# GiboDidact/Computational_ray_tracer

Hardware: AMD Instinct MI355X
Metric: Msamples/s (whole node) at 1920x1080; achieved HBM GB/s vs roofline (higher is better)
Workload: dtype f32; 1 GPU; BASELINE configs[1]: Cornell box 1920x1080 @ 256 spp (16x16 stratified jittered), diffuse + NEE, max depth 5, 1 quad light, 36 triangles; spp_total=256, max_depth=5, parallelism=pixel-tile shards x1 (32x32 tiles) + RCCL film reduce

## Files before the change

### computational_ray_tracer_amd/csrc/rt_host.cpp

```cpp
#include <algorithm>
#include <cstddef>
#include <cstdlib>
#include <cmath>
#include <cstdio>
#include <cstring>
#include <initializer_list>
#include <limits>
#include <queue>
#include <string>
#include <thread>
#include <utility>
#include <vector>

#include "../../include/rtmi355x.h"
#include "../data/spectra_data.h"
#include "../data/sensor_data.h"
#include "rt_devbuf.h"
#include "rt_guard.h"
#include "rt_internal.h"
#include "rt_texture.h"

using namespace rtmi;

namespace {
// ... 431 lines not shown
    hipStream_t stream = nullptr;
    hipEvent_t film_done = nullptr;
};

struct Knobs {
    bool stage_events = true;
    int lanes = kDefaultLanes;
    int shadow_queue = 0;
    int shadow_dfs = 1;
    int sort_rays = 1;
    float bvh_node_cost = 2.5f;
    int bvh_max_leaf = kBvhMaxLeaf;
    float bvh_any_cost = 2.f;
    int bvh_any_leaf = 4;
    int force_amb = -1;
    int coop = 1;
    int mat_bins = 1;
    int emit_filter = 1;
    int debug_path = 0;
    int sort_dir_bits = 3, sort_org_bits = 3;
    int sort_org_major = -1;
    int sort_nee = 1, sort_nee_bits = 8;
    int hit_compact = 1;
    size_t batch_samples = 0;
    int denoise_lds = 1;
};

static Knobs read_knobs() {
    Knobs k;
    if (std::getenv("RTMI_NO_STAGE_EVENTS")) k.stage_events = false;
    if (const char* e = std::getenv("RTMI_LANES")) k.lanes = std::max(1, std::min(kLanes, std::atoi(e)));
    if (const char* e = std::getenv("RTMI_SHADOW_QUEUE")) k.shadow_queue = std::atoi(e);
    if (const char* e = std::getenv("RTMI_SHADOW_DFS")) k.shadow_dfs = std::atoi(e);
    if (const char* e = std::getenv("RTMI_SORT")) k.sort_rays = std::atoi(e);
    if (const char* e = std::getenv("RTMI_BVH_CI")) k.bvh_node_cost = (float)std::atof(e);
    if (const char* e = std::getenv("RTMI_BVH_LEAF")) k.bvh_max_leaf = std::max(1, std::min(15, std::atoi(e)));
    if (const char* e = std::getenv("RTMI_BVH_ANY")) {
        float ac;
        int al;
        if (std::sscanf(e, "%f/%d", &ac, &al) == 2) {
            k.bvh_any_cost = ac;
            k.bvh_any_leaf = std::max(1, std::min(15, al));
        }
    }
    if (const char* e = std::getenv("RTMI_FORCE_AMB")) k.force_amb = std::max(-1, std::min(30, std::atoi(e)));
    if (const char* e = std::getenv("RTMI_COOP")) k.coop = std::atoi(e) != 0;
    if (const char* e = std::getenv("RTMI_MAT_BINS")) k.mat_bins = std::atoi(e);
    if (const char* e = std::getenv("RTMI_EMIT_FILTER")) k.emit_filter = std::atoi(e);
    if (const char* e = std::getenv("RTMI_DEBUG_PATH_KERNELS")) k.debug_path = std::atoi(e) != 0;
    if (const char* e = std::getenv("RTMI_SORT_BITS")) {
        int db = 3, ob = 4, om = -1;
        const int got = std::sscanf(e, "%d/%d/%d", &db, &ob, &om);
        if (got >= 2 && db >= 0 && db <= 9 && ob >= 0 && ob <= 9 && 3 + 2 * db + 3 * ob <= 32) {
            k.sort_dir_bits = db;
            k.sort_org_bits = ob;
            if (got == 3) k.sort_org_major = om < 0 ? -1 : (om ? 1 : 0);
        }
    }
    if (const char* e = std::getenv("RTMI_SORT_NEE")) std::sscanf(e, "%d/%d", &k.sort_nee, &k.sort_nee_bits);
    k.sort_nee_bits = std::max(1, std::min(9, k.sort_nee_bits));
    if (const char* e = std::getenv("RTMI_HIT_COMPACT")) k.hit_compact = std::atoi(e) != 0;
    if (const char* e = std::getenv("RTMI_BATCH_SAMPLES")) k.batch_samples = (size_t)std::max(0L, std::atol(e));
    if (const char* e = std::getenv("RTMI_DENOISE_LDS")) k.denoise_lds = std::atoi(e) != 0;
    return k;
}

struct rt_ctx {
    float4 sort_lo{}, sort_scale{};
    int device = 0;
    int octree_build = RT_OCTREE_BUILD_DEVICE;
    hipStream_t stream = nullptr;
    std::string err;
    bool have_scene = false, have_cam = false, have_smp = false, have_film = false, have_integ = false;
    rt_camera_desc cam{};
    rt_sampler_desc smp{};
    rt_film_desc film{};
    rt_integrator_desc integ{};
    int n_tris = 0;
    std::vector<float> h_bounds;
    std::vector<int32_t> h_child, h_leaf_first, h_leaf_count, h_refs;
    rt_octree_info info{};
    bool cull = false;
    bool scene_full = false;
    DevScene dsc{};
// ... 152 lines not shown
    HIPCHK(c, b.shLA.reserve(n)); HIPCHK(c, b.shLB.reserve(n));
    return RT_OK;
}

int ensure_sort_workspace(rt_ctx* c, Batch& b, size_t n) {
    HIPCHK(c, b.sRay.reserve(2 * n)); HIPCHK(c, b.sS.reserve(n));
    HIPCHK(c, b.sVals.reserve(n)); HIPCHK(c, b.sValsAlt.reserve(n));
    HIPCHK(c, b.sKeys.reserve(n)); HIPCHK(c, b.sKeysAlt.reserve(n)); HIPCHK(c, b.sQKey.reserve(n));
    HIPCHK(c, b.sTemp.reserve(sort_temp_bytes()));
    return RT_OK;
}

int ensure_ring(rt_ctx* c, Work& w) {
    if (c->dsc.qcap != 0) return RT_OK;
    HIPCHK(c, w.ring.reserve((size_t)c->dsc.ring_threads * (size_t)(c->dsc.ring_mask + 1)));
    return RT_OK;
}
DevScene lane_scene(const rt_ctx* c, const Work& w) {
    DevScene d = c->dsc;
    d.ring = w.ring.get();
    return d;
}

int ensure_workspace(rt_ctx* c, Work& w, size_t n, bool path) {
    int rc;
    HIPCHK(c, w.qcount.reserve(2 * kQRegion));
    if (&w != &c->ws[0] && !w.stream) HIPCHK(c, hipStreamCreateWithFlags(&w.stream, hipStreamNonBlocking));
    if (!w.film_done) HIPCHK(c, hipEventCreateWithFlags(&w.film_done, hipEventDisableTiming));
    if ((rc = ensure_ring(c, w))) return rc;
    Batch& b = w.b;
    const bool hit_d = path && c->knobs.hit_compact && c->dsc.qcap == 1 && !c->dsc.full;
    if (b.capacity(path) >= n) {
        if (hit_d) HIPCHK(c, b.hitD.reserve(n));
        return RT_OK;
    }
    b = Batch{};
    size_t nq = path ? 2 * n : n;
    HIPCHK(c, b.ray.reserve(2 * nq));
    HIPCHK(c, b.pdfA.reserve(n)); HIPCHK(c, b.pdfB.reserve(n));
    HIPCHK(c, b.hitB.reserve(n)); HIPCHK(c, b.hitPrim.reserve(n));
    if (path) {
        HIPCHK(c, b.rec.reserve((size_t)kRecF4 * n));
        if (hit_d) HIPCHK(c, b.hitD.reserve(n));
    } else {
        HIPCHK(c, b.lamA.reserve(n)); HIPCHK(c, b.lamB.reserve(n));
    }
    return RT_OK;
}

static int dim_get2d(const DevSampler& S, int dim) {
    if (S.kind == 1) return dim + 2;
    if (S.kind == 2) return (dim + 1 >= kSobolDims ? 2 : dim) + 2;
    return dim;
}
static int dim_after_camera(const DevSampler& S, const DevCamera& cam) {
    int dim = S.kind == 2 ? 2 : 0;
// ... 359 lines not shown
            int nIdx = std::min(B, ie - b0);
            int nS = nIdx * n_work;
            SampleIds ids = sample_ids(work, n_work, b0);
            RefIO r = ref_io(c, w.b, nS, nsh);
            hipEvent_t e0 = ev_start(c, st);
            HIPCHK(c, launch_generate(st, c->grid, nS, ids, cam, smp, fd, r.go));
            ev_mark(c, st, ST_GEN, e0);
            e0 = ev_start(c, st);
            HIPCHK(c, launch_trace_closest(st, 0, c->dsc.qcap, lane_scene(c, w), r.tio, d_ctr));
            ev_mark(c, st, ST_TRACE, e0);
            r.sio.work_pixels = work; r.sio.n_pixels = n_work; r.sio.n_index = nIdx;
            r.sio.film = film;
            r.sio.mom = pass.mom;
            e0 = ev_start(c, st);
            HIPCHK(c, launch_ref_shade_film(st, 0, c->dsc, d_spec, fd, r.sio, d_ctr));
            ev_mark(c, st, ST_FILM, e0);
        }
        return RT_OK;
    }

    const int nbatch = (ie - ib + B - 1) / B;
    const int lanes = std::max(1, std::min(std::min(kn.lanes, kLanes), nbatch));
    const bool sort_rays = c->dsc.qcap != 1 && kn.sort_rays;
    for (int l = 0; l < lanes; ++l) {
        if ((rc = ensure_workspace(c, c->ws[l], ncap, true))) return rc;
        if (sort_rays && (rc = ensure_sort_workspace(c, c->ws[l].b, ncap))) return rc;
        if (c->dsc.qcap != 1) HIPCHK(c, c->ws[l].tfb.reserve(ncap));
    }
    const bool dyn = c->dsc.qcap != 1;
    const int lean = c->dsc.full ? 2 : 1;
    const bool shq = c->dsc.qcap != 1 && !c->dsc.full;
    if (shq)
        for (int l = 0; l < lanes; ++l)
            if ((rc = ensure_shadow_workspace(c, c->ws[l].b, ncap))) return rc;
    const bool nee = c->dsc.full && c->dsc.n_lights > 0;
    if (nee)
        for (int l = 0; l < lanes; ++l)
            if ((rc = ensure_nee_workspace(c, c->ws[l].b, nmax * (size_t)nee_stride(c->dsc.n_lights), ncap))) return rc;
    const bool bins = nee && c->dsc.qcap != 1 && kn.mat_bins;
    const int grid = c->grid;
    auto lstream = [&](int l) { return l == 0 ? st : c->ws[l].stream; };
    if (lanes > 1) {
        HIPCHK(c, hipEventRecord(c->ws[0].film_done, st));
        for (int l = 1; l < lanes; ++l) HIPCHK(c, hipStreamWaitEvent(c->ws[l].stream, c->ws[0].film_done, 0));
    }
    const size_t qs = ncap;
    const bool records = c->dsc.qcap != 1;
    const size_t rec_fs = records ? 1 : nmax;
// ... 31 lines not shown
                int nxt = cur[l] ^ 1;
                const float4* cO = b.rayO() + 2 * (size_t)cur[l] * qs;
                const float4* cD = cO + 1;
                int* qc_cur = w.qcount.get() + kQRegion * cur[l];
                int* qc_nxt = w.qcount.get() + kQRegion * nxt;
                const bool efilter = kn.emit_filter && c->dsc.full && depth == c->integ.max_depth && depth > 0 &&
                                     c->dsc.n_emit_tris >= 0;
                if (efilter) HIPCHK(c, hipMemsetAsync(qc_nxt, 0, kQRegion * sizeof(int), s));
                hipEvent_t e0;
                QueueView qv = depth == 0 ? QueueView{nullptr, Sq[l], nSq[l], nsh}
                                          : QueueView{qc_cur + kQLen, Sq[l], 0, nsh};
                const DevScene dsl = lane_scene(c, w);
                if (efilter) {
                    const EmitIO eio{qv, cO, b.rayO() + 2 * (size_t)nxt * qs, qc_nxt + kQLen};
                    e0 = ev_start(c, s);
                    HIPCHK(c, launch_emitter_filter(s, grid, dsl, eio));
                    ev_mark(c, s, ST_FILTER, e0);
                    cO = eio.nO;
                    cD = cO + 1;
                    qv = QueueView{qc_nxt + kQLen, Sq[l], 0, nsh};
                }
                TraceIO tio{cO, cD, qv, 0, b.hitB.get(), b.hitPrim.get(), dyn ? qc_cur + kQTraceTicket : nullptr, 1};
                if (depth > 0 && !efilter) tio.zero = qc_nxt;
                const bool hitc = kn.hit_compact && c->dsc.qcap == 1 && !c->dsc.full && depth > 0;
                if (hitc) {
                    tio.hq_d = b.hitD.get();
                    tio.hq_len = qc_cur + kQShadowLen;
                }
                if (c->dsc.qcap != 1) {
                    tio.fb_pos = w.tfb.get();
                    tio.fb_len = qc_cur + kQTraceFallback;
                }
                const NeeSlots ns = nee ? b.nee : NeeSlots{};
                BinIO bio{qv, b.hitPrim.get(), {}, qc_cur + kQBinLen};
                for (int cl = 0; cl < kMatClasses; ++cl) bio.idx[cl] = ns.bin[cl];
                if (depth == 0) { bio.rayO = cO; bio.rec = rv; }
                if (sort_rays && depth > 0 && !efilter) {
                    SortRaysIO so{b.sQKey.get(), b.sS.get(), b.sKeys.get(), b.sKeysAlt.get(), b.sVals.get(),
                                  b.sValsAlt.get(), b.sTemp.get(), kn.sort_dir_bits, kn.sort_org_bits, qc_cur + kQLen,
                                  Sq[l]};
                    e0 = ev_start(c, s);
                    HIPCHK(c, launch_sort_rays(s, so));
                    ev_mark(c, s, ST_SORT, e0);
                    tio.perm = b.sS.get();
                    tio.so = b.sRay.get();
                    cO = tio.so; cD = cO + 1;
                }
                e0 = ev_start(c, s);
                HIPCHK(c, launch_trace_closest(s, grid, c->dsc.qcap, dsl, tio, d_ctr));
// ... 34 lines not shown
                    sqio.defer = kn.shadow_queue ? 0 : 1;
                }
                NeeIO nio{};
                const bool sort_nee = nee && sort_rays && kn.sort_nee;
                if (nee)
                    nio = NeeIO{b.neeRec.get(), ns.queue, qc_cur + kQShadowLen, qc_cur + kQShadowTicket, ns.fallback,
                                qc_cur + kQNeeFallback, sort_nee ? ns.key : nullptr, c->sort_lo, c->sort_scale,
                                kn.sort_nee_bits};
                if (c->tx.live) nio.tex = c->tx.dev.get();
                nio.ml = c->ml.any ? 1 : 0;
                e0 = ev_start(c, s);
                if (bins) {
                    HIPCHK(c, launch_bin_materials(s, grid, dsl, bio));
                    for (int cl = 0; cl < kMatClasses; ++cl) {
                        PathIO bp = pio;
                        bp.q = QueueView{qc_cur + kQBinLen + cl * kShards * kQStride, Sq[l], 0, nsh};
                        bp.ticket = qc_cur + kQBinTicket + cl * kShards * kQStride;
                        bp.bin_idx = bio.idx[cl];
                        HIPCHK(c, launch_path_shade(s, grid, c->dsc.qcap, dsl, d_spec, smp, fd, ids, bp, d_ctr,
                                                    sqio, nio, 1 + cl));
                    }
                } else {
                    HIPCHK(c, launch_path_shade(s, grid, c->dsc.qcap, dsl, d_spec, smp, fd, ids, pio, d_ctr, sqio,
                                                nio));
                }
                ev_mark(c, s, ST_SHADE, e0);
                if (sort_nee) {
                    SortNeeIO so{ns.queue, qc_cur + kQShadowLen, Sq[l], ns.key, b.sKeys.get(), b.sKeysAlt.get(),
                                 b.sVals.get(), b.sValsAlt.get(), b.sTemp.get(), kn.sort_nee_bits};
                    e0 = ev_start(c, s);
                    HIPCHK(c, launch_sort_nee(s, so));
                    ev_mark(c, s, ST_SORT, e0);
                }
                if (nee) {
                    e0 = ev_start(c, s);
                    HIPCHK(c, launch_path_nee(s, grid, c->dsc.qcap, dsl, d_spec, pio, nio, d_ctr));
                    if (c->dsc.qcap != 1 && !c->dsc.coop_ok)
                        HIPCHK(c, launch_path_nee_fallback(s, grid, c->dsc.qcap, dsl, d_spec, pio, nio, d_ctr));
                    ev_mark(c, s, ST_SHADOW, e0);
                }
                if (shq && !(sqio.defer && c->dsc.coop_ok)) {
                    e0 = ev_start(c, s);
                    HIPCHK(c, launch_path_shadow(s, grid, c->dsc.qcap, kn.shadow_dfs != 0, dsl, pio, sqio, d_ctr));
                    ev_mark(c, s, ST_SHADOW, e0);
                }
                cur[l] = nxt;
            }
// ... 2539 lines not shown
```

### computational_ray_tracer_amd/csrc/rt_internal.h

```cpp
#pragma once
#include <hip/hip_runtime.h>
#include <stdint.h>

#include <vector>

namespace rtmi {

static const int kSpecN = 471;
static const int kF1Max = 128;

struct DevSpectra {
    float X[kSpecN], Y[kSpecN], Z[kSpecN], D65[kSpecN];
    float f1_lambda[kF1Max], f1_value[kF1Max];
    int f1_n;
    float bk7_lambda[kF1Max], bk7_value[kF1Max];
    int bk7_n;
    float SR[kSpecN], SG[kSpecN], SB[kSpecN];
    float4 SPK[kSpecN];
};

struct DevCamera {
    float r2c[16], c2w[16];
    float lens_radius, focal_distance;
    int type;
// ... 192 lines not shown

static const int kShards = 8;
static const int kQStride = 64;
enum { kQLen = 0, kQTraceTicket = 1 * kShards * kQStride, kQShadeTicket = 2 * kShards * kQStride,
       kQShadowLen = 3 * kShards * kQStride, kQShadowTicket = 4 * kShards * kQStride,
       kQNeeFallback = 5 * kShards * kQStride,
       kQBinLen = 6 * kShards * kQStride, kQBinTicket = 8 * kShards * kQStride,
       kQTraceFallback = 10 * kShards * kQStride,
       kQRegion = 11 * kShards * kQStride };
static const int kMatClasses = 2;
inline __host__ __device__ int shard_stride(int n, int ns) {
    int s = (n + ns - 1) / ns;
    return (s + 63) & ~63;
}
struct QueueView {
    const int* len;
    int S;
    int n;
    int ns;
};
static const int kBlockThreads = 256;
static const int kClusterTris = 2;

struct TraceIO {
    const float4* rayO; const float4* rayD;
    QueueView q;
    int set;
    float4* hitB;
    int* hitPrim;
    int* ticket = nullptr;
    int rsh = 0;
    const int* perm = nullptr;
    float4* so = nullptr;
    int* fb_pos = nullptr;
    int* fb_len = nullptr;
    int* zero = nullptr;
    float4* hq_d = nullptr;
    int* hq_len = nullptr;
};

struct BinIO {
    QueueView q;
    const int* hitPrim;
    int* idx[kMatClasses];
    int* len;
    const float4* rayO = nullptr;
    RecView rec{};
};
hipError_t launch_bin_materials(hipStream_t st, int grid, const DevScene& sc, const BinIO& io);

struct EmitIO {
    QueueView q;
    const float4* rayO;
    float4* nO;
// ... 116 lines not shown
size_t sort_temp_bytes();
hipError_t launch_sort_rays(hipStream_t st, const SortRaysIO& io);
struct SortNeeIO {
    int* slot; int* len; int S;
    const unsigned* key;
    unsigned* keys; unsigned* keys_alt; int* vals; int* vals_alt;
    void* temp;
    int org_bits;
};
hipError_t launch_sort_nee(hipStream_t st, const SortNeeIO& io);
hipError_t launch_oct_classify(hipStream_t st, int nnodes, const float* cbox, const int* seg, const int* ent,
                               const float* tri9, unsigned char* mask, int* stats);
hipError_t launch_oct_scatter(hipStream_t st, int njobs, int nchild, const int* job, const int* ent,
                              const unsigned char* mask, int* ent_next, int* s0);
hipError_t launch_ref_shade_film(hipStream_t st, int grid, const DevScene& sc, const DevSpectra* sp, const DevFilm& film,
                                 const ShadeRefIO& io, unsigned long long* ctr);
hipError_t launch_records(hipStream_t st, const DevScene& sc, const DevSpectra* sp, const DevFilm& film,
                          const ShadeRefIO& sio, const RecordIO& io);
hipError_t launch_path_shadow(hipStream_t st, int grid, int qcap, bool dfs, const DevScene& sc, const PathIO& io,
                              const ShadowQueueIO& shq, unsigned long long* ctr);
hipError_t launch_path_shade(hipStream_t st, int grid, int qcap, const DevScene& sc, const DevSpectra* sp,
                             const DevSampler& smp, const DevFilm& film, const SampleIds& ids, const PathIO& io,
                             unsigned long long* ctr, const ShadowQueueIO& shq = ShadowQueueIO{},
                             const NeeIO& nee = NeeIO{}, int matclass = 0);
hipError_t launch_path_film(hipStream_t st, int grid, const DevSpectra* sp, const DevFilm& film, const PathFilmIO& io,
                            unsigned long long* ctr);
hipError_t launch_path_nee_fallback(hipStream_t st, int grid, int qcap, const DevScene& sc, const DevSpectra* sp,
                                    const PathIO& io, const NeeIO& nee, unsigned long long* ctr);
hipError_t launch_path_nee(hipStream_t st, int grid, int qcap, const DevScene& sc, const DevSpectra* sp,
                           const PathIO& io, const NeeIO& nee, unsigned long long* ctr);
hipError_t launch_resolve(hipStream_t st, int n, const float4* film, const float* m_xyz_from_sensor,
                          const float* m_rgb_from_xyz, unsigned char* out, int srgb);
hipError_t launch_film_gather(hipStream_t st, int n, const int* work, const float4* film, float4* out);
hipError_t launch_film_scatter(hipStream_t st, int n, const int* work, const float4* in, float4* film);

struct AdaptiveIO {
    int res_x, res_y;
    const float4* film;
    const float2* mom;
    float rel_error, abs_floor;
    float* block_error;
    int* converged;
    int* totals;
};
hipError_t launch_adaptive_error(hipStream_t st, const AdaptiveIO& io);
inline __host__ __device__ int adaptive_waves(int n) { return (n + 63) / 64; }
hipError_t launch_adaptive_compact(hipStream_t st, const AdaptiveIO& io, const int* in, int n, int* out,
// ... 100 lines not shown
```

### computational_ray_tracer_amd/csrc/rt_kernels.hip

```cpp
#include <hip/hip_runtime.h>

#include <mutex>
#include <type_traits>
#include <unordered_map>
#include <utility>

#include "rt_device.h"

namespace rtmi {

static constexpr int kBlock = kBlockThreads;
static constexpr int kLeafChunk = 32;
static constexpr int kLdsQ = 32;
static constexpr int kTriUnroll = 4;
#ifndef RT_BVH_STACK
#define RT_BVH_STACK 16
#endif
static constexpr int kBvhStack = RT_BVH_STACK;
__shared__ uint2 g_bstk[kBvhStack * kBlock];
static_assert(sizeof(uint2) * kBvhStack >= 2 * kLdsQ, "the BFS FIFO lives in the BVH stack's LDS");
#ifndef RT_ANY_STACK
#define RT_ANY_STACK 24
#endif
static constexpr int kAnyStack = RT_ANY_STACK;
// ... 24 lines not shown
    if constexpr (QCAP == 1) {
        stage_leaf1(sc, set);
    } else {
        const float4* b = sc.bvh[ANY ? kBvhAny : set];
        if (b)
            for (int i = threadIdx.x; i < kBvhNodeRead * kBvhTopNodes; i += blockDim.x)
                g_top[i] = b[(i / kBvhNodeRead) * kBvhNodeF4 + i % kBvhNodeRead];
        simd_init();
        __syncthreads();
    }
}
struct BvhNode8 {
    float4 N0;
    uint4 N1, QX, QY, QZ;
};
__device__ __forceinline__ uint4 as_u4(float4 v) {
    return make_uint4(__float_as_uint(v.x), __float_as_uint(v.y), __float_as_uint(v.z), __float_as_uint(v.w));
}
__device__ __forceinline__ BvhNode8 load_node8(const float4* __restrict__ nodes, int node) {
    const float4* N = node < kBvhTopNodes ? g_top + kBvhNodeRead * node : nodes + (size_t)kBvhNodeF4 * node;
    return BvhNode8{N[0], as_u4(N[1]), as_u4(N[2]), as_u4(N[3]), as_u4(N[4])};
}
__shared__ float4 g_tri1[4 * 64];
__device__ __forceinline__ bool stage_tris1(const DevScene& sc) {
    const bool ok = sc.n_tris <= 64;
    if (ok)
        for (int i = threadIdx.x; i < sc.n_tris; i += blockDim.x) {
            g_tri1[4 * i] = sc.triWorld[3 * i];
            g_tri1[4 * i + 1] = sc.triWorld[3 * i + 1];
            g_tri1[4 * i + 2] = sc.triWorld[3 * i + 2];
            const DevMaterial dm = sc.materials[sc.triMaterial[i]];
            g_tri1[4 * i + 3] = make_float4(dm.c0, dm.c1, dm.c2, dm.emit);
        }
    __syncthreads();
    return ok;
}
static constexpr int kLdsMats = 64;
__shared__ DevMaterial g_mat[kLdsMats];
__device__ __forceinline__ bool stage_materials(const DevScene& sc) {
    const bool ok = sc.n_materials <= kLdsMats;
    if (ok)
        for (int i = threadIdx.x; i < sc.n_materials; i += blockDim.x) g_mat[i] = sc.materials[i];
    __syncthreads();
    return ok;
}
__device__ __forceinline__ DevMaterial mat_at(const DevScene& sc, bool lds, int m) {
    if (lds) return g_mat[m];
    return sc.materials[m];
}
__device__ __forceinline__ int mbcnt64(uint64_t m) {
    return (int)__builtin_amdgcn_mbcnt_hi((uint32_t)(m >> 32), __builtin_amdgcn_mbcnt_lo((uint32_t)m, 0u));
}
__device__ __forceinline__ void wave_lds_sync() {
    __builtin_amdgcn_fence(__ATOMIC_RELEASE, "wavefront");
    __builtin_amdgcn_wave_barrier();
    __builtin_amdgcn_fence(__ATOMIC_ACQUIRE, "wavefront");
}

// ... 1305 lines not shown
        for (int si = 0; si < sc.n_shapes; ++si) {
            DevShape sh = ldconst(sc.shapes, si);
            V3 ph;
            float th;
            if (shape_isect<CULL>(sh, v3(o4.x, o4.y, o4.z), v3(d4.x, d4.y, d4.z), tm, ph, th)) {
                prim = sc.n_tris + si; b0 = ph.x; b1 = ph.y; b2 = ph.z; t = th; tm = th;
            }
        }
    }
}
template <bool CULL>
__device__ __forceinline__ int finish_closest(const DevScene& sc, const TraceIO& io, int p, float4 o4, float4 d4,
                                              int prim, float b0, float b1, float b2, float t) {
    closest_shapes<CULL>(sc, o4, d4, prim, b0, b1, b2, t);
    io.hitB[p] = make_float4(b0, b1, b2, t);
    io.hitPrim[p] = prim;
    return prim;
}

#ifndef RT_TRACE_KZ
#define RT_TRACE_KZ 1
#endif

template <int QCAP, bool FBL, bool HQ = false>
__global__ void __launch_bounds__(kBlock) RT_WAVES_ATTR(QCAP) k_trace_closest(DevScene sc, TraceIO io, unsigned long long* ctr) {
    stage_scene<QCAP, false>(sc, io.set);
    if (io.zero && blockIdx.x == 0)
        for (int i = threadIdx.x; i < kQRegion; i += blockDim.x) io.zero[i] = 0;
    ctr_t nn = 0, nt = 0, nh = 0, nr = 0, nfb = 0, novf = 0;
    auto trace_one = [&](int p, float4 o4, float4 d4) __attribute__((always_inline)) {
        float b0 = 0, b1 = 0, b2 = 0, t = 0;
        int prim;
        if constexpr (QCAP != 1 && FBL) {
            bool amb = false;
            prim = traverse_bvh<false, RT_TRACE_KZ != 0>(sc, io.set, v3(o4.x, o4.y, o4.z), v3(d4.x, d4.y, d4.z),
                                                         3.402823466e+38f, b0, b1, b2, t, nn, nt, amb);
            if (amb) {
                ++nfb;
                io.fb_pos[atomicAdd(io.fb_len, 1)] = p;
                return;
            }
        } else {
            prim = traverse_any<QCAP, false>(sc, io.set, v3(o4.x, o4.y, o4.z), v3(d4.x, d4.y, d4.z), 3.402823466e+38f,
                                             b0, b1, b2, t, nn, nt, nfb);
        }
        prim = finish_closest<QCAP != 1>(sc, io, p, o4, d4, prim, b0, b1, b2, t);
        nh += prim >= 0;
        nr += 1;
    };
    if constexpr (HQ) {
        static_assert(QCAP == 1 && kStaticItems == 2, "a chunk's first record is parked, its second appends both");
        __shared__ int hq_lds[2 * (kBlock / 64) + 1];
        const int n = q_len(io.q, 0);
        int k = blockIdx.x * kChunk + (int)threadIdx.x;
        float4 o4 = make_float4(0, 0, 0, 0), d4 = o4;
        if (k < n) { o4 = io.rayO[k << io.rsh]; d4 = io.rayD[k << io.rsh]; }
        float4 rb0 = o4, rd0 = o4;
        for (int c = blockIdx.x; c * kChunk < n; c += gridDim.x) {
#pragma unroll 1
            for (int r = 0; r < kStaticItems; ++r) {
                const int kn = r + 1 < kStaticItems ? k + kBlock : (c + (int)gridDim.x) * kChunk + (int)threadIdx.x;
                float4 on = o4, dn = d4;
                if (kn < n) { on = io.rayO[kn << io.rsh]; dn = io.rayD[kn << io.rsh]; }
                float b0 = 0, b1 = 0, b2 = 0, t = 0;
                int prim = -1;
                if (k < n) {
                    prim = traverse_any<QCAP, false>(sc, io.set, v3(o4.x, o4.y, o4.z), v3(d4.x, d4.y, d4.z),
                                                     3.402823466e+38f, b0, b1, b2, t, nn, nt, nfb);
                    closest_shapes<false>(sc, o4, d4, prim, b0, b1, b2, t);
                    nh += prim >= 0;
                    nr += 1;
                }
                const float4 rb = make_float4(b0, b1, b2, o4.w), rd = make_float4(d4.x, d4.y, d4.z, __int_as_float(prim));
                if (r == 0) {
                    rb0 = rb;
                    rd0 = rd;
                } else {
                    const bool h0 = __float_as_int(rd0.w) >= 0;
                    int p0, p1;
                    block_append2(io.hq_len, h0, prim >= 0, hq_lds, p0, p1);
                    if (h0) { io.hitB[p0] = rb0; io.hq_d[p0] = rd0; }
                    if (prim >= 0) { io.hitB[p1] = rb; io.hq_d[p1] = rd; }
                }
                k = kn; o4 = on; d4 = dn;
            }
        }
    } else if (!io.ticket && io.q.ns == 1) {
        const int n = q_len(io.q, 0);
        auto item = [&](int i) {
            return (blockIdx.x + (i / kStaticItems) * gridDim.x) * kChunk + (i % kStaticItems) * kBlock +
                   (int)threadIdx.x;
        };
        int k = item(0);
        float4 o4 = make_float4(0, 0, 0, 0), d4 = o4;
        if (k < n) { o4 = io.rayO[k << io.rsh]; d4 = io.rayD[k << io.rsh]; }
        for (int i = 1; k < n; ++i) {
            const int kn = item(i);
            float4 on = o4, dn = d4;
            if (kn < n) { on = io.rayO[kn << io.rsh]; dn = io.rayD[kn << io.rsh]; }
            trace_one(k, o4, d4);
            k = kn; o4 = on; d4 = dn;
        }
    } else if (!io.ticket) {
        StaticChunks ch(io.q);
        int base;
        while (ch.next(base)) {
#pragma unroll 1
            for (int r = 0; r < kStaticItems; ++r) {
                const int idx = base + r * kBlock + (int)threadIdx.x;
                if (idx < ch.len) {
// ... 313 lines not shown
__device__ __forceinline__ void shadow_push(const ShadowQueueIO& shq, int pos, V3 so, V3 sd, float stmax, int slot,
                                            const float Ld[8]) {
    shq.shO[pos] = make_float4(so.x, so.y, so.z, stmax);
    shq.shD[pos] = make_float4(sd.x, sd.y, sd.z, __int_as_float(slot));
    shq.shLA[pos] = make_float4(Ld[0], Ld[1], Ld[2], Ld[3]);
    shq.shLB[pos] = make_float4(Ld[4], Ld[5], Ld[6], Ld[7]);
}
__device__ __forceinline__ void shadow_ld(const ShadowQueueIO& shq, int k, float Ld[8]) {
    load8(shq.shLA, shq.shLB, k, Ld);
}
__device__ __forceinline__ void add_to_L(const RecView& rec, int slot, const float Ld[8], bool zero_first) {
    float L[8];
    rload8_or_zero(rec, slot, R_L, L, zero_first);
#pragma unroll
    for (int i = 0; i < 8; ++i) L[i] += Ld[i];
    rstore8(rec, slot, R_L, L);
}
__device__ __forceinline__ void push_bounce(const PathIO& io, int pos, float4 nO, float4 nD, int slot) {
    nO.w = __int_as_float(slot);
    io.nO[2 * pos] = nO; io.nD[2 * pos] = nD;
    if (io.nkey.key) io.nkey.key[pos] = ray_sort_key(nO, nD, io.nkey);
}

template <int QCAP, bool HQ = false>
__global__ void __launch_bounds__(kBlock) __attribute__((amdgpu_waves_per_eu(QCAP == 1 ? RT_SHADE1_WAVES : RT_SHADE_WAVES))) k_path_shade(DevScene sc, const DevSpectra* sp, DevSampler smp,
                                                                         DevFilm film, SampleIds ids, PathIO io,
                                                                         unsigned long long* ctr, ShadowQueueIO shq) {
    const float InvPi = 0.31830988618379067154f;
    bool lds_tris = false;
    stage_spectra(sp);
    stage_scene<QCAP>(sc, 0);
    if constexpr (QCAP == 1) lds_tris = stage_tris1(sc);
    __shared__ int lds[2 * (kBlock / 64) + 1];
    __shared__ float4 pend[QCAP == 1 ? 2 * kBlock : 1];
    bool pend0 = false;
    ctr_t snn = 0, snt = 0, nsh = 0, sfb = 0, novf = 0;
    const bool d0 = io.lean && io.depth == 0;
    constexpr bool WAVE = QCAP != 1;
    std::conditional_t<QCAP == 1, QueueItemsOne, QueueItems<WAVE>> items(io.ticket, io.q);
    int qj, qidx;
    bool live;
    while (items.next(qj, qidx, live)) {
        const int k = qj * io.q.S + qidx;
        bool wantShadow = false, wantNext = false, storedL = false;
        float4 nO = make_float4(0, 0, 0, 0), nD = nO;
        V3 so = v3(0, 0, 0), sd = so;
        float stmax = 0.f;
        float Ld[8];
        int slot = -1;
        if (live) {
            int prim;
            float4 hq = make_float4(0, 0, 0, 0), hd = hq;
            if constexpr (HQ) {
                hq = io.hitB[k];
                hd = io.hq_d[k];
                slot = __float_as_int(hq.w);
                prim = __float_as_int(hd.w);
            } else {
                slot = io.depth == 0 ? k : __float_as_int(io.rayO[2 * k].w);
                prim = io.hitPrim[k];
            }
            if (HQ || prim >= 0) {
                float lam[8], beta[8];
                rload8(io.rec, slot, R_LAM, lam);
                if (d0) {
#pragma unroll
                    for (int i = 0; i < 8; ++i) beta[i] = 1.f;
                } else {
                    rload8(io.rec, slot, R_BETA, beta);
                }
                float4 P0, P1, P2, mt;
                if (QCAP == 1 && lds_tris) {
                    P0 = g_tri1[4 * prim]; P1 = g_tri1[4 * prim + 1]; P2 = g_tri1[4 * prim + 2]; mt = g_tri1[4 * prim + 3];
                } else {
                    P0 = sc.triWorld[3 * prim]; P1 = sc.triWorld[3 * prim + 1]; P2 = sc.triWorld[3 * prim + 2];
                    const DevMaterial dm = sc.materials[sc.triMaterial[prim]];
                    mt = make_float4(dm.c0, dm.c1, dm.c2, dm.emit);
                }
                V3 p0 = v3(P0.x, P0.y, P0.z), p1 = v3(P1.x, P1.y, P1.z), p2 = v3(P2.x, P2.y, P2.z);
                V3 ng = vnorm(vcross(vsub(p0, p2), vsub(p1, p2)));
                const float4 d4 = HQ ? hd : io.rayD[2 * k];
                V3 rayd = vnorm(v3(d4.x, d4.y, d4.z));
                if (mt.w > 0) {
                    if (io.depth == 0 && vdot(ng, rayd) < 0) {
                        float L[8];
                        rload8_or_zero(io.rec, slot, R_L, L, d0);
#pragma unroll
                        for (int i = 0; i < 8; ++i) L[i] += beta[i] * (mt.w * d65_query(sp, lam[i]));
                        rstore8(io.rec, slot, R_L, L);
                        storedL = true;
                    }
                } else if (io.depth < io.max_depth) {
                    V3 nrm = ng;
                    if (vdot(nrm, rayd) > 0) nrm = v3(-nrm.x, -nrm.y, -nrm.z);
                    const float4 hb = HQ ? hq : io.hitB[k];
                    V3 p = vadd(vadd(vmul(p0, hb.x), vmul(p1, hb.y)), vmul(p2, hb.z));
                    float off = 1e-4f * (1.0f + max3f(fabsf(p.x), fabsf(p.y), fabsf(p.z)));
                    V3 po = vadd(p, vmul(nrm, off));
                    constexpr bool kLate = QCAP == 1;
                    float R[8], le = 0.f, wgt = 0.f;
                    if constexpr (!kLate) {
#pragma unroll
                        for (int i = 0; i < 8; ++i) R[i] = sigmoid_eval(mt.x, mt.y, mt.z, lam[i]);
                    }
                    Smp sm;
                    restore_sampler(ids, film, io, slot, sm, smp.kind, smp.seed);
                    float u0, u1;
                    sm.get2d(smp, u0, u1);
                    if (sc.n_lights > 0) {
                        const DevLight& Lq = sc.light0;
                        V3 pl = vadd(vadd(v3(Lq.p[0], Lq.p[1], Lq.p[2]), vmul(v3(Lq.e1[0], Lq.e1[1], Lq.e1[2]), u0)),
                                     vmul(v3(Lq.e2[0], Lq.e2[1], Lq.e2[2]), u1));
                        V3 wv = vsub(pl, po);
                        float dist2 = vdot(wv, wv);
                        float dist = sqrtf(dist2);
                        V3 wi = vmul(wv, 1.0f / dist);
                        float cs = vdot(nrm, wi);
                        float cl = -vdot(v3(Lq.n[0], Lq.n[1], Lq.n[2]), wi);
// ... 771 lines not shown
hipError_t launch_emitter_filter(hipStream_t st, int grid, const DevScene& sc, const EmitIO& io) {
    if (sc.n_emit_tris < 0 || sc.n_emit_tris > kMaxEmitTris) return hipErrorInvalidValue;
    hipLaunchKernelGGL(k_emitter_filter, dim3(grid_for(io.q.n ? io.q.n : grid * kBlock, grid)), dim3(kBlock), 0, st,
                       sc, io);
    return hipGetLastError();
}

hipError_t launch_generate(hipStream_t st, int grid, int nS, const SampleIds& ids, const DevCamera& cam,
                           const DevSampler& smp, const DevFilm& film, const GenOut& out) {
    hipLaunchKernelGGL(k_generate, dim3(grid_for(nS, grid)), dim3(kBlock), 0, st, nS, ids, cam, smp, film, out);
    return hipGetLastError();
}

hipError_t launch_trace_closest(hipStream_t st, int grid, int qcap, const DevScene& sc, const TraceIO& io,
                                unsigned long long* ctr) {
    const int gb = ring_clamp(grid_for(io.q.len ? grid * kBlock : io.q.n, grid), qcap, sc);
    const bool fbl = io.fb_pos != nullptr;
    if (fbl && (!io.fb_len || qcap == 1)) return hipErrorInvalidValue;
    void (*k)(DevScene, TraceIO, unsigned long long*);
    switch (qcap) {
        case 0: k = fbl ? k_trace_closest<0, true> : k_trace_closest<0, false>; break;
        case 1:
            if (io.hq_len) {
                if (io.ticket || io.q.ns != 1 || !io.hq_d) return hipErrorInvalidValue;
                k = k_trace_closest<1, false, true>;
            } else {
                k = k_trace_closest<1, false>;
            }
            break;
        case 16: k = fbl ? k_trace_closest<16, true> : k_trace_closest<16, false>; break;
        default: return hipErrorInvalidValue;
    }
    return launch_resident(k, gb, grid, st, sc, io, ctr);
}

hipError_t launch_trace_fallback(hipStream_t st, int grid, int qcap, const DevScene& sc, const TraceIO& io,
                                 unsigned long long* ctr) {
    if (!io.fb_pos || !io.fb_len) return hipErrorInvalidValue;
    const int gb = ring_clamp(std::min(grid > 0 ? grid : 1, kFallbackBlocks), qcap, sc);
    switch (qcap) {
        case 0: return launch_resident(k_trace_fallback<0>, gb, grid, st, sc, io, ctr);
        case 16: return launch_resident(k_trace_fallback<16>, gb, grid, st, sc, io, ctr);
        default: return hipErrorInvalidValue;
    }
}

hipError_t launch_ref_shade_film(hipStream_t st, int grid, const DevScene& sc, const DevSpectra* sp, const DevFilm& film,
                                 const ShadeRefIO& io, unsigned long long* ctr) {
// ... 8 lines not shown
                          const ShadeRefIO& sio, const RecordIO& io) {
    hipLaunchKernelGGL(k_records, dim3(grid_for(io.n, 0)), dim3(kBlock), 0, st, sc, sp, film, sio, io);
    return hipGetLastError();
}


hipError_t launch_path_shadow(hipStream_t st, int grid, int qcap, bool dfs, const DevScene& sc, const PathIO& io,
                              const ShadowQueueIO& shq, unsigned long long* ctr) {
    int gb = grid > 0 ? grid : 1;
    if (shq.defer) gb = std::min(gb, kFallbackBlocks);
    gb = ring_clamp(gb, qcap, sc);
    const int v = !shq.defer && sc.coop_ok ? 2 : dfs ? 1 : 0;
    void (*k)(DevScene, PathIO, ShadowQueueIO, unsigned long long*);
    switch (qcap) {
        case 0: k = v == 2 ? k_path_shadow<0, false, true> : v == 1 ? k_path_shadow<0, true> : k_path_shadow<0, false>; break;
        case 16: k = v == 2 ? k_path_shadow<16, false, true> : v == 1 ? k_path_shadow<16, true> : k_path_shadow<16, false>; break;
        default: return hipErrorInvalidValue;
    }
    return launch_resident(k, gb, grid, st, sc, io, shq, ctr);
}

hipError_t launch_path_shade(hipStream_t st, int grid, int qcap, const DevScene& sc, const DevSpectra* sp,
                             const DevSampler& smp, const DevFilm& film, const SampleIds& ids, const PathIO& io,
                             unsigned long long* ctr, const ShadowQueueIO& shq, const NeeIO& nee, int matclass) {
    const int gb = ring_clamp(grid > 0 ? grid : 1, qcap, sc);
    if (sc.full && sc.n_lights > 0 && !nee.rec) return hipErrorInvalidValue;
    if (!sc.full && qcap != 1 && !shq.shO) return hipErrorInvalidValue;
    if (sc.full) {
        void (*k)(DevScene, const DevSpectra*, DevSampler, DevFilm, SampleIds, PathIO, NeeIO);
        const int v = (nee.tex ? 1 : 0) | (nee.ml ? 2 : 0);
#define RT_SHADE_FULL(Q, M) \
    (v == 0 ? k_path_shade_full<Q, M> : v == 1 ? k_path_shade_full<Q, M, true> : v == 2 ? k_path_shade_full<Q, M, false, true> \
                                                                                       : k_path_shade_full<Q, M, true, true>)
        switch (qcap) {
            case 0: k = matclass == 1 ? RT_SHADE_FULL(0, 1) : matclass == 2 ? RT_SHADE_FULL(0, 2) : RT_SHADE_FULL(0, 0); break;
            case 1: k = RT_SHADE_FULL(1, 0); break;
            case 16: k = matclass == 1 ? RT_SHADE_FULL(16, 1) : matclass == 2 ? RT_SHADE_FULL(16, 2) : RT_SHADE_FULL(16, 0); break;
            default: return hipErrorInvalidValue;
        }
#undef RT_SHADE_FULL
        return launch_resident(k, gb, grid, st, sc, sp, smp, film, ids, io, nee);
    }
    void (*k)(DevScene, const DevSpectra*, DevSampler, DevFilm, SampleIds, PathIO, unsigned long long*, ShadowQueueIO);
    switch (qcap) {
        case 0: k = k_path_shade<0>; break;
        case 1: k = io.hq_d ? k_path_shade<1, true> : k_path_shade<1>; break;
        case 16: k = k_path_shade<16>; break;
        default: return hipErrorInvalidValue;
    }
    return launch_resident(k, gb, grid, st, sc, sp, smp, film, ids, io, ctr, shq);
}

hipError_t launch_path_nee(hipStream_t st, int grid, int qcap, const DevScene& sc, const DevSpectra* sp,
                           const PathIO& io, const NeeIO& nee, unsigned long long* ctr) {
    const int gb = ring_clamp(grid > 0 ? grid : 1, qcap, sc);
    if (qcap != 1 && (!nee.fb_slot || !nee.fb_len)) return hipErrorInvalidValue;
    void (*k)(DevScene, const DevSpectra*, PathIO, NeeIO, unsigned long long*);
    const int v = (nee.tex ? 1 : 0) | (nee.ml ? 2 : 0);
#define RT_NEE(Q) \
    (v == 0 ? k_path_nee<Q, false> : v == 1 ? k_path_nee<Q, false, true> : v == 2 ? k_path_nee<Q, false, false, true> \
                                                                              : k_path_nee<Q, false, true, true>)
    switch (qcap) {
        case 0: k = RT_NEE(0); break;
        case 1: k = RT_NEE(1); break;
        case 16: k = RT_NEE(16); break;
        default: return hipErrorInvalidValue;
    }
#undef RT_NEE
    return launch_resident(k, gb, grid, st, sc, sp, io, nee, ctr);
// ... 67 lines not shown
```

Before: 2290 Msamples/s.

## Pack hit records into one word to drop ray-direction reads

After: 2335 Msamples/s, median of 6. 2.0% higher.

```diff
diff --git a/computational_ray_tracer_amd/csrc/rt_host.cpp b/computational_ray_tracer_amd/csrc/rt_host.cpp
--- a/computational_ray_tracer_amd/csrc/rt_host.cpp
+++ b/computational_ray_tracer_amd/csrc/rt_host.cpp
@@ -477,6 +477,7 @@
     int sort_org_major = -1;
     int sort_nee = 1, sort_nee_bits = 8;
     int hit_compact = 1;
+    int hit_pack = 1;
     size_t batch_samples = 0;
     int denoise_lds = 1;
 };
@@ -515,6 +516,7 @@
     if (const char* e = std::getenv("RTMI_SORT_NEE")) std::sscanf(e, "%d/%d", &k.sort_nee, &k.sort_nee_bits);
     k.sort_nee_bits = std::max(1, std::min(9, k.sort_nee_bits));
     if (const char* e = std::getenv("RTMI_HIT_COMPACT")) k.hit_compact = std::atoi(e) != 0;
+    if (const char* e = std::getenv("RTMI_HIT_PACK")) k.hit_pack = std::atoi(e) != 0;
     if (const char* e = std::getenv("RTMI_BATCH_SAMPLES")) k.batch_samples = (size_t)std::max(0L, std::atol(e));
     if (const char* e = std::getenv("RTMI_DENOISE_LDS")) k.denoise_lds = std::atoi(e) != 0;
     return k;
@@ -713,16 +715,22 @@
     return d;
 }
 
-int ensure_workspace(rt_ctx* c, Work& w, size_t n, bool path) {
+bool hit_pack_active(const rt_ctx* c, size_t nmax) {
+    return c->knobs.hit_pack && c->knobs.hit_compact && c->dsc.qcap == 1 && !c->dsc.full &&
+           c->dsc.n_tris <= kHitPackTris && nmax <= (size_t)kHitPackSlots;
+}
+
+int ensure_workspace(rt_ctx* c, Work& w, size_t n, bool path, bool hit_pack = false) {
     int rc;
     HIPCHK(c, w.qcount.reserve(2 * kQRegion));
     if (&w != &c->ws[0] && !w.stream) HIPCHK(c, hipStreamCreateWithFlags(&w.stream, hipStreamNonBlocking));
     if (!w.film_done) HIPCHK(c, hipEventCreateWithFlags(&w.film_done, hipEventDisableTiming));
     if ((rc = ensure_ring(c, w))) return rc;
     Batch& b = w.b;
-    const bool hit_d = path && c->knobs.hit_compact && c->dsc.qcap == 1 && !c->dsc.full;
+    const bool hit_d = path && c->knobs.hit_compact && c->dsc.qcap == 1 && !c->dsc.full && !hit_pack;
     if (b.capacity(path) >= n) {
         if (hit_d) HIPCHK(c, b.hitD.reserve(n));
+        else if (path) b.hitD.reset();
         return RT_OK;
     }
     b = Batch{};
@@ -1128,8 +1136,9 @@
     const int nbatch = (ie - ib + B - 1) / B;
     const int lanes = std::max(1, std::min(std::min(kn.lanes, kLanes), nbatch));
     const bool sort_rays = c->dsc.qcap != 1 && kn.sort_rays;
+    const bool hpack = hit_pack_active(c, nmax);
     for (int l = 0; l < lanes; ++l) {
-        if ((rc = ensure_workspace(c, c->ws[l], ncap, true))) return rc;
+        if ((rc = ensure_workspace(c, c->ws[l], ncap, true, hpack))) return rc;
         if (sort_rays && (rc = ensure_sort_workspace(c, c->ws[l].b, ncap))) return rc;
         if (c->dsc.qcap != 1) HIPCHK(c, c->ws[l].tfb.reserve(ncap));
     }
@@ -1207,9 +1216,11 @@
                 }
                 TraceIO tio{cO, cD, qv, 0, b.hitB.get(), b.hitPrim.get(), dyn ? qc_cur + kQTraceTicket : nullptr, 1};
                 if (depth > 0 && !efilter) tio.zero = qc_nxt;
+                if (hpack && depth == 0) tio.hq_pack = 1;
                 const bool hitc = kn.hit_compact && c->dsc.qcap == 1 && !c->dsc.full && depth > 0;
                 if (hitc) {
-                    tio.hq_d = b.hitD.get();
+                    if (hpack) tio.hq_pack = 1;
+                    else tio.hq_d = b.hitD.get();
                     tio.hq_len = qc_cur + kQShadowLen;
                 }
                 if (c->dsc.qcap != 1) {
@@ -1290,7 +1301,7 @@
                     }
                 } else {
                     HIPCHK(c, launch_path_shade(s, grid, c->dsc.qcap, dsl, d_spec, smp, fd, ids, pio, d_ctr, sqio,
-                                                nio));
+                                                nio, 0, hpack));
                 }
                 ev_mark(c, s, ST_SHADE, e0);
                 if (sort_nee) {
diff --git a/computational_ray_tracer_amd/csrc/rt_internal.h b/computational_ray_tracer_amd/csrc/rt_internal.h
--- a/computational_ray_tracer_amd/csrc/rt_internal.h
+++ b/computational_ray_tracer_amd/csrc/rt_internal.h
@@ -238,6 +238,46 @@
 static const int kBlockThreads = 256;
 static const int kClusterTris = 2;
 
+static const int kHitPackSlots = 1 << 24;
+static const int kHitPackTris = 64;
+inline __host__ __device__ constexpr unsigned hit_pack(int slot, int prim, bool facing) {
+    return (unsigned)slot | (unsigned)prim << 24 | (facing ? 1u << 30 : 0u);
+}
+struct HitWord {
+    int slot, prim;
+    bool facing;
+};
+inline __host__ __device__ constexpr HitWord hit_unpack(unsigned w) {
+    return HitWord{(int)(w & (unsigned)(kHitPackSlots - 1)), (int)(w >> 24 & (unsigned)(kHitPackTris - 1)),
+                   (w >> 30 & 1u) != 0};
+}
+inline __host__ __device__ constexpr unsigned hit_pack0(int prim, bool flip, bool front) {
+    return (unsigned)prim | (front ? 1u << 29 : 0u) | (flip ? 1u << 30 : 0u);
+}
+struct HitWord0 {
+    int prim;
+    bool flip, front;
+};
+inline __host__ __device__ constexpr HitWord0 hit_unpack0(unsigned w) {
+    return HitWord0{(int)w < 0 ? -1 : (int)(w & (unsigned)(kHitPackTris - 1)), (w >> 30 & 1u) != 0, (w >> 29 & 1u) != 0};
+}
+static_assert(hit_unpack0(hit_pack0(kHitPackTris - 1, true, false)).prim == kHitPackTris - 1 &&
+                  hit_unpack0(hit_pack0(kHitPackTris - 1, true, false)).flip &&
+                  !hit_unpack0(hit_pack0(kHitPackTris - 1, true, false)).front &&
+                  hit_unpack0(hit_pack0(0, false, true)).front && !hit_unpack0(hit_pack0(0, false, true)).flip &&
+                  hit_unpack0(0xffffffffu).prim == -1 && (hit_pack0(kHitPackTris - 1, true, true) >> 31) == 0,
+              "packed depth-0 hit word: round trip, a negative word is a miss");
+static_assert(hit_unpack(hit_pack(kHitPackSlots - 1, kHitPackTris - 1, true)).slot == kHitPackSlots - 1 &&
+                  hit_unpack(hit_pack(kHitPackSlots - 1, kHitPackTris - 1, true)).prim == kHitPackTris - 1 &&
+                  hit_unpack(hit_pack(kHitPackSlots - 1, kHitPackTris - 1, true)).facing,
+              "packed hit word: round trip at the field limits, facing set");
+static_assert(hit_unpack(hit_pack(kHitPackSlots - 1, kHitPackTris - 1, false)).slot == kHitPackSlots - 1 &&
+                  hit_unpack(hit_pack(kHitPackSlots - 1, kHitPackTris - 1, false)).prim == kHitPackTris - 1 &&
+                  !hit_unpack(hit_pack(kHitPackSlots - 1, kHitPackTris - 1, false)).facing,
+              "packed hit word: round trip at the field limits, facing clear");
+static_assert((hit_pack(kHitPackSlots - 1, kHitPackTris - 1, true) >> 31) == 0 && hit_unpack(hit_pack(0, 0, false)).slot == 0,
+              "packed hit word: bit 31 stays clear (a negative word marks a miss)");
+
 struct TraceIO {
     const float4* rayO; const float4* rayD;
     QueueView q;
@@ -246,6 +286,7 @@
     int* hitPrim;
     int* ticket = nullptr;
     int rsh = 0;
+    int hq_pack = 0;
     const int* perm = nullptr;
     float4* so = nullptr;
     int* fb_pos = nullptr;
@@ -408,7 +449,7 @@
 hipError_t launch_path_shade(hipStream_t st, int grid, int qcap, const DevScene& sc, const DevSpectra* sp,
                              const DevSampler& smp, const DevFilm& film, const SampleIds& ids, const PathIO& io,
                              unsigned long long* ctr, const ShadowQueueIO& shq = ShadowQueueIO{},
-                             const NeeIO& nee = NeeIO{}, int matclass = 0);
+                             const NeeIO& nee = NeeIO{}, int matclass = 0, bool hit_pack = false);
 hipError_t launch_path_film(hipStream_t st, int grid, const DevSpectra* sp, const DevFilm& film, const PathFilmIO& io,
                             unsigned long long* ctr);
 hipError_t launch_path_nee_fallback(hipStream_t st, int grid, int qcap, const DevScene& sc, const DevSpectra* sp,
diff --git a/computational_ray_tracer_amd/csrc/rt_kernels.hip b/computational_ray_tracer_amd/csrc/rt_kernels.hip
--- a/computational_ray_tracer_amd/csrc/rt_kernels.hip
+++ b/computational_ray_tracer_amd/csrc/rt_kernels.hip
@@ -70,18 +70,38 @@
     return BvhNode8{N[0], as_u4(N[1]), as_u4(N[2]), as_u4(N[3]), as_u4(N[4])};
 }
 __shared__ float4 g_tri1[4 * 64];
+__device__ __forceinline__ V3 tri_face_normal(V3 p0, V3 p1, V3 p2) { return vnorm(vcross(vsub(p0, p2), vsub(p1, p2))); }
+template <bool NG = false>
 __device__ __forceinline__ bool stage_tris1(const DevScene& sc) {
     const bool ok = sc.n_tris <= 64;
     if (ok)
         for (int i = threadIdx.x; i < sc.n_tris; i += blockDim.x) {
-            g_tri1[4 * i] = sc.triWorld[3 * i];
-            g_tri1[4 * i + 1] = sc.triWorld[3 * i + 1];
-            g_tri1[4 * i + 2] = sc.triWorld[3 * i + 2];
+            if constexpr (NG) {
+                float4 P0 = sc.triWorld[3 * i], P1 = sc.triWorld[3 * i + 1], P2 = sc.triWorld[3 * i + 2];
+                const V3 ng = tri_face_normal(v3(P0.x, P0.y, P0.z), v3(P1.x, P1.y, P1.z), v3(P2.x, P2.y, P2.z));
+                P0.w = ng.x; P1.w = ng.y; P2.w = ng.z;
+                g_tri1[4 * i] = P0;
+                g_tri1[4 * i + 1] = P1;
+                g_tri1[4 * i + 2] = P2;
+            } else {
+                g_tri1[4 * i] = sc.triWorld[3 * i];
+                g_tri1[4 * i + 1] = sc.triWorld[3 * i + 1];
+                g_tri1[4 * i + 2] = sc.triWorld[3 * i + 2];
+            }
             const DevMaterial dm = sc.materials[sc.triMaterial[i]];
             g_tri1[4 * i + 3] = make_float4(dm.c0, dm.c1, dm.c2, dm.emit);
         }
     __syncthreads();
     return ok;
+}
+__shared__ float4 g_ng1[kHitPackTris];
+__device__ __forceinline__ void stage_ng1(const DevScene& sc) {
+    for (int i = threadIdx.x; i < sc.n_tris && i < kHitPackTris; i += blockDim.x) {
+        const float4 P0 = sc.triWorld[3 * i], P1 = sc.triWorld[3 * i + 1], P2 = sc.triWorld[3 * i + 2];
+        const V3 ng = tri_face_normal(v3(P0.x, P0.y, P0.z), v3(P1.x, P1.y, P1.z), v3(P2.x, P2.y, P2.z));
+        g_ng1[i] = make_float4(ng.x, ng.y, ng.z, 0.f);
+    }
+    __syncthreads();
 }
 static constexpr int kLdsMats = 64;
 __shared__ DevMaterial g_mat[kLdsMats];
@@ -1433,9 +1453,11 @@
 #define RT_TRACE_KZ 1
 #endif
 
-template <int QCAP, bool FBL, bool HQ = false>
+template <int QCAP, bool FBL, bool HQ = false, bool PK = false>
 __global__ void __launch_bounds__(kBlock) RT_WAVES_ATTR(QCAP) k_trace_closest(DevScene sc, TraceIO io, unsigned long long* ctr) {
+    static_assert(!PK || (QCAP == 1 && !FBL), "packed records exist on the single-leaf simple path only");
     stage_scene<QCAP, false>(sc, io.set);
+    if constexpr (PK) stage_ng1(sc);
     if (io.zero && blockIdx.x == 0)
         for (int i = threadIdx.x; i < kQRegion; i += blockDim.x) io.zero[i] = 0;
     ctr_t nn = 0, nt = 0, nh = 0, nr = 0, nfb = 0, novf = 0;
@@ -1455,7 +1477,18 @@
             prim = traverse_any<QCAP, false>(sc, io.set, v3(o4.x, o4.y, o4.z), v3(d4.x, d4.y, d4.z), 3.402823466e+38f,
                                              b0, b1, b2, t, nn, nt, nfb);
         }
-        prim = finish_closest<QCAP != 1>(sc, io, p, o4, d4, prim, b0, b1, b2, t);
+        if constexpr (PK) {
+            closest_shapes<false>(sc, o4, d4, prim, b0, b1, b2, t);
+            int w = -1;
+            if (prim >= 0) {
+                const float4 n4 = g_ng1[prim];
+                const float dn = vdot(v3(n4.x, n4.y, n4.z), vnorm(v3(d4.x, d4.y, d4.z)));
+                w = (int)hit_pack0(prim, dn > 0, dn < 0);
+            }
+            io.hitB[p] = make_float4(b0, b1, b2, __int_as_float(w));
+        } else {
+            prim = finish_closest<QCAP != 1>(sc, io, p, o4, d4, prim, b0, b1, b2, t);
+        }
         nh += prim >= 0;
         nr += 1;
     };
@@ -1482,21 +1515,37 @@
                     nh += prim >= 0;
                     nr += 1;
                 }
-                const float4 rb = make_float4(b0, b1, b2, o4.w), rd = make_float4(d4.x, d4.y, d4.z, __int_as_float(prim));
+                float4 rb = make_float4(b0, b1, b2, o4.w);
+                const float4 rd = make_float4(d4.x, d4.y, d4.z, __int_as_float(prim));
+                if constexpr (PK) {
+                    int w = -1;
+                    if (prim >= 0) {
+                        const float4 n4 = g_ng1[prim];
+                        const bool facing = vdot(v3(n4.x, n4.y, n4.z), vnorm(v3(d4.x, d4.y, d4.z))) > 0;
+                        w = (int)hit_pack(__float_as_int(o4.w), prim, facing);
+                    }
+                    rb.w = __int_as_float(w);
+                }
                 if (r == 0) {
                     rb0 = rb;
                     rd0 = rd;
                 } else {
-                    const bool h0 = __float_as_int(rd0.w) >= 0;
+                    const bool h0 = __float_as_int(PK ? rb0.w : rd0.w) >= 0;
                     int p0, p1;
                     block_append2(io.hq_len, h0, prim >= 0, hq_lds, p0, p1);
-                    if (h0) { io.hitB[p0] = rb0; io.hq_d[p0] = rd0; }
-                    if (prim >= 0) { io.hitB[p1] = rb; io.hq_d[p1] = rd; }
+                    if (h0) {
+                        io.hitB[p0] = rb0;
+                        if constexpr (!PK) io.hq_d[p0] = rd0;
+                    }
+                    if (prim >= 0) {
+                        io.hitB[p1] = rb;
+                        if constexpr (!PK) io.hq_d[p1] = rd;
+                    }
                 }
                 k = kn; o4 = on; d4 = dn;
             }
         }
-    } else if (!io.ticket && io.q.ns == 1) {
+    } else if (PK || (!io.ticket && io.q.ns == 1)) {
         const int n = q_len(io.q, 0);
         auto item = [&](int i) {
             return (blockIdx.x + (i / kStaticItems) * gridDim.x) * kChunk + (i % kStaticItems) * kBlock +
@@ -1856,7 +1905,7 @@
     if (io.nkey.key) io.nkey.key[pos] = ray_sort_key(nO, nD, io.nkey);
 }
 
-template <int QCAP, bool HQ = false>
+template <int QCAP, bool HQ = false, bool PK = false>
 __global__ void __launch_bounds__(kBlock) __attribute__((amdgpu_waves_per_eu(QCAP == 1 ? RT_SHADE1_WAVES : RT_SHADE_WAVES))) k_path_shade(DevScene sc, const DevSpectra* sp, DevSampler smp,
                                                                          DevFilm film, SampleIds ids, PathIO io,
                                                                          unsigned long long* ctr, ShadowQueueIO shq) {
@@ -1864,7 +1913,8 @@
     bool lds_tris = false;
     stage_spectra(sp);
     stage_scene<QCAP>(sc, 0);
-    if constexpr (QCAP == 1) lds_tris = stage_tris1(sc);
+    static_assert(!PK || QCAP == 1, "packed records exist on the single-leaf simple path only");
+    if constexpr (QCAP == 1) lds_tris = stage_tris1<PK>(sc);
     __shared__ int lds[2 * (kBlock / 64) + 1];
     __shared__ float4 pend[QCAP == 1 ? 2 * kBlock : 1];
     bool pend0 = false;
@@ -1885,7 +1935,21 @@
         if (live) {
             int prim;
             float4 hq = make_float4(0, 0, 0, 0), hd = hq;
-            if constexpr (HQ) {
+            bool facing = false, front = false;
+            if constexpr (PK && !HQ) {
+                hq = io.hitB[k];
+                const HitWord0 hw = hit_unpack0(__float_as_uint(hq.w));
+                slot = k;
+                prim = hw.prim;
+                facing = hw.flip;
+                front = hw.front;
+            } else if constexpr (PK) {
+                hq = io.hitB[k];
+                const HitWord hw = hit_unpack(__float_as_uint(hq.w));
+                slot = hw.slot;
+                prim = hw.prim;
+                facing = hw.facing;
+            } else if constexpr (HQ) {
                 hq = io.hitB[k];
                 hd = io.hq_d[k];
                 slot = __float_as_int(hq.w);
@@ -1904,7 +1968,7 @@
                     rload8(io.rec, slot, R_BETA, beta);
                 }
                 float4 P0, P1, P2, mt;
-                if (QCAP == 1 && lds_tris) {
+                if (QCAP == 1 && (PK || lds_tris)) {
                     P0 = g_tri1[4 * prim]; P1 = g_tri1[4 * prim + 1]; P2 = g_tri1[4 * prim + 2]; mt = g_tri1[4 * prim + 3];
                 } else {
                     P0 = sc.triWorld[3 * prim]; P1 = sc.triWorld[3 * prim + 1]; P2 = sc.triWorld[3 * prim + 2];
@@ -1912,11 +1976,16 @@
                     mt = make_float4(dm.c0, dm.c1, dm.c2, dm.emit);
                 }
                 V3 p0 = v3(P0.x, P0.y, P0.z), p1 = v3(P1.x, P1.y, P1.z), p2 = v3(P2.x, P2.y, P2.z);
-                V3 ng = vnorm(vcross(vsub(p0, p2), vsub(p1, p2)));
-                const float4 d4 = HQ ? hd : io.rayD[2 * k];
-                V3 rayd = vnorm(v3(d4.x, d4.y, d4.z));
+                V3 ng, rayd = v3(0, 0, 0);
+                if constexpr (PK) {
+                    ng = v3(P0.w, P1.w, P2.w);
+                } else {
+                    ng = tri_face_normal(p0, p1, p2);
+                    const float4 d4 = HQ ? hd : io.rayD[2 * k];
+                    rayd = vnorm(v3(d4.x, d4.y, d4.z));
+                }
                 if (mt.w > 0) {
-                    if (io.depth == 0 && vdot(ng, rayd) < 0) {
+                    if (!(PK && HQ) && io.depth == 0 && (PK ? front : vdot(ng, rayd) < 0)) {
                         float L[8];
                         rload8_or_zero(io.rec, slot, R_L, L, d0);
 #pragma unroll
@@ -1926,8 +1995,8 @@
                     }
                 } else if (io.depth < io.max_depth) {
                     V3 nrm = ng;
-                    if (vdot(nrm, rayd) > 0) nrm = v3(-nrm.x, -nrm.y, -nrm.z);
-                    const float4 hb = HQ ? hq : io.hitB[k];
+                    if (PK ? facing : vdot(nrm, rayd) > 0) nrm = v3(-nrm.x, -nrm.y, -nrm.z);
+                    const float4 hb = HQ || PK ? hq : io.hitB[k];
                     V3 p = vadd(vadd(vmul(p0, hb.x), vmul(p1, hb.y)), vmul(p2, hb.z));
                     float off = 1e-4f * (1.0f + max3f(fabsf(p.x), fabsf(p.y), fabsf(p.z)));
                     V3 po = vadd(p, vmul(nrm, off));
@@ -2745,8 +2814,12 @@
         case 0: k = fbl ? k_trace_closest<0, true> : k_trace_closest<0, false>; break;
         case 1:
             if (io.hq_len) {
-                if (io.ticket || io.q.ns != 1 || !io.hq_d) return hipErrorInvalidValue;
-                k = k_trace_closest<1, false, true>;
+                if (io.ticket || io.q.ns != 1) return hipErrorInvalidValue;
+                if (io.hq_pack ? sc.n_tris > kHitPackTris : !io.hq_d) return hipErrorInvalidValue;
+                k = io.hq_pack ? k_trace_closest<1, false, true, true> : k_trace_closest<1, false, true>;
+            } else if (io.hq_pack) {
+                if (io.ticket || io.q.ns != 1 || io.q.len || sc.n_tris > kHitPackTris) return hipErrorInvalidValue;
+                k = k_trace_closest<1, false, false, true>;
             } else {
                 k = k_trace_closest<1, false>;
             }
@@ -2801,8 +2874,11 @@
 
 hipError_t launch_path_shade(hipStream_t st, int grid, int qcap, const DevScene& sc, const DevSpectra* sp,
                              const DevSampler& smp, const DevFilm& film, const SampleIds& ids, const PathIO& io,
-                             unsigned long long* ctr, const ShadowQueueIO& shq, const NeeIO& nee, int matclass) {
+                             unsigned long long* ctr, const ShadowQueueIO& shq, const NeeIO& nee, int matclass,
+                             bool hit_pack) {
     const int gb = ring_clamp(grid > 0 ? grid : 1, qcap, sc);
+    if (hit_pack && (qcap != 1 || sc.full || io.ticket || sc.n_tris > kHitPackTris || (io.depth == 0 && io.q.len)))
+        return hipErrorInvalidValue;
     if (sc.full && sc.n_lights > 0 && !nee.rec) return hipErrorInvalidValue;
     if (!sc.full && qcap != 1 && !shq.shO) return hipErrorInvalidValue;
     if (sc.full) {
@@ -2823,7 +2899,10 @@
     void (*k)(DevScene, const DevSpectra*, DevSampler, DevFilm, SampleIds, PathIO, unsigned long long*, ShadowQueueIO);
     switch (qcap) {
         case 0: k = k_path_shade<0>; break;
-        case 1: k = io.hq_d ? k_path_shade<1, true> : k_path_shade<1>; break;
+        case 1:
+            k = hit_pack ? (io.depth == 0 ? k_path_shade<1, false, true> : k_path_shade<1, true, true>)
+                         : io.hq_d ? k_path_shade<1, true> : k_path_shade<1>;
+            break;
         case 16: k = k_path_shade<16>; break;
         default: return hipErrorInvalidValue;
     }
```
